# Veeryan/FDTD-solver-antennas

Measured on AMD Instinct MI355X. Metric: Mcells/s (Yee cells x steps / s), higher is better.
Workload: dtype f32; 1 GPU; NS: 300x300x60 2.45 GHz patch on FR-4 (fixed scene), CPML-10, 1 lumped port(s), NF2FF surfaces (record); cells=5400000, operator=classes, parallelism=single GPU, fields_finite=True

## Files before the change

### fdtd-solver-antennas_amd/_capi.py

```python
from __future__ import annotations

import ctypes as C
import os
from typing import Optional

import numpy as np

_HERE = os.path.dirname(os.path.abspath(__file__))
HIP_LIB_NAME = "libfdtd_hip.so"

ABI_SYMBOLS = [
    "fdtd_version", "fdtd_device_count", "fdtd_backend", "fdtd_create", "fdtd_destroy",
    "fdtd_last_error", "fdtd_set_operator_raw", "fdtd_set_operator_classes", "fdtd_build_operator",
    "fdtd_operator_form", "fdtd_get_operator", "fdtd_set_cpml",
    "fdtd_set_mur", "fdtd_set_signal", "fdtd_add_source", "fdtd_add_probe", "fdtd_get_probe",
    "fdtd_set_dft", "fdtd_add_dft_box", "fdtd_get_dft_box", "fdtd_set_recorder", "fdtd_rec_transform", "fdtd_run", "fdtd_run_profiled",
    "fdtd_get_step", "fdtd_energy", "fdtd_p2p_export", "fdtd_p2p_attach", "fdtd_p2p_selftest", "fdtd_p2p_detach", "fdtd_p2p_link_info", "fdtd_schedule_info", "fdtd_comm_unique_id", "fdtd_comm_init", "fdtd_comm_nranks", "fdtd_link", "fdtd_run_linked", "fdtd_half_step",
    "fdtd_halo_get", "fdtd_halo_put", "fdtd_get_field", "fdtd_set_field", "fdtd_farfield",
]

SHEET_SYMBOLS = ["fdtd_sheet_set", "fdtd_sheet_get"]
SHEET_MAX_K = 8
DEBYE_SYMBOLS = ["fdtd_debye_set", "fdtd_debye_get"]
DEBYE_MAX_K = 8
DEBYE_MAX_MEDIA = 8
LORENTZ_SYMBOLS = ["fdtd_lorentz_set", "fdtd_lorentz_get"]
LORENTZ_MAX_K = 4
LORENTZ_MAX_MEDIA = 8
LUMPED_SYMBOLS = ["fdtd_lumped_set", "fdtd_lumped_get"]
MAGNETIC_SYMBOLS = ["fdtd_magnetic_set", "fdtd_magnetic_get"]
MAGNETIC_MAX_CLASSES = 255
TRAFFIC_SYMBOLS = ["fdtd_traffic_info"]
VOXEL_SYMBOLS = ["fdtd_voxelize"]
CONFORMAL_SYMBOLS = ["fdtd_conformal_set", "fdtd_conformal_get", "fdtd_voxel_fractions"]
SAR_SYMBOLS = ["fdtd_sar_local", "fdtd_sar_average"]
PLANEWAVE_SYMBOLS = ["fdtd_planewave_set"]
MAX_BOXES = 64


class FdtdDesc(C.Structure):
    _fields_ = [("nx", C.c_int32), ("ny", C.c_int32), ("nz", C.c_int32),
                ("k0", C.c_int32), ("nk", C.c_int32),
                ("rank", C.c_int32), ("world", C.c_int32),
                ("device", C.c_int32), ("max_steps", C.c_int32),
                ("flags", C.c_uint32), ("dt", C.c_double)]


class FdtdProfile(C.Structure):
    _fields_ = [("ms_total", C.c_double), ("ms_update_e", C.c_double), ("ms_update_h", C.c_double),
                ("launches_e", C.c_int32), ("launches_h", C.c_int32),
                ("steps", C.c_int32), ("fused", C.c_int32), ("ms_event_overhead", C.c_double)]


FLAG_KERNEL_AUTO, FLAG_KERNEL_DIRECT, FLAG_KERNEL_WAVEFRONT, FLAG_KERNEL_RESIDENT, FLAG_KERNEL_MASK = 0, 1, 5, 6, 0xF
FLAG_OVERLAP_ON, FLAG_OVERLAP_OFF, FLAG_LOOPBACK = 0x20, 0x40, 0x80
KIND_V, KIND_I = 0, 1
PHASE_E, PHASE_H = 0, 1
HALO_H_UP, HALO_E_DOWN = 0, 1

_vp, _i, _i64p = C.c_void_p, C.c_int, C.POINTER(C.c_int64)


def bind(lib: C.CDLL) -> C.CDLL:
    p = C.c_void_p
    sig = {
        "fdtd_version": (C.c_int, []),
# ... 90 lines not shown
        "fdtd_magnetic_get": (C.c_int, [p, C.c_int, p, p]),
    }
    assert sorted(magnetic_sig) == sorted(MAGNETIC_SYMBOLS)
    for name, (res, args) in magnetic_sig.items():
        fn = getattr(lib, name, None)
        if fn is not None:
            fn.restype = res
            fn.argtypes = args
    traffic_sig = {"fdtd_traffic_info": (C.c_int, [p, p, C.POINTER(C.c_int32), C.POINTER(C.c_int64)])}
    assert sorted(traffic_sig) == sorted(TRAFFIC_SYMBOLS)
    for name, (res, args) in traffic_sig.items():
        fn = getattr(lib, name, None)
        if fn is not None:
            fn.restype = res
            fn.argtypes = args
    voxel_sig = {
        "fdtd_voxelize": (C.c_int, [C.c_int, C.c_int, C.c_int, C.c_int, p, C.c_int, p, C.c_int, p, C.c_double, p, p]),
    }
    assert sorted(voxel_sig) == sorted(VOXEL_SYMBOLS)
    for name, (res, args) in voxel_sig.items():
        fn = getattr(lib, name, None)
        if fn is not None:
            fn.restype = res
            fn.argtypes = args
    conformal_sig = {
        "fdtd_conformal_set": (C.c_int, [p, C.c_int, p, p, p]),
        "fdtd_conformal_get": (C.c_int, [p, p, p]),
        "fdtd_voxel_fractions": (C.c_int, [C.c_int, C.c_int, C.c_int, C.c_int, p, C.c_int, p, C.c_int, p, C.c_double, C.c_double,
                                           C.c_int, p, C.c_int64, p, p, p]),
    }
# ... 29 lines not shown

def has_planewave(lib: C.CDLL) -> bool:
    return all(hasattr(lib, n) for n in PLANEWAVE_SYMBOLS)


def has_conformal(lib: C.CDLL) -> bool:
    return all(hasattr(lib, n) for n in CONFORMAL_SYMBOLS)


def has_voxelize(lib: C.CDLL) -> bool:
    return all(hasattr(lib, n) for n in VOXEL_SYMBOLS)


def has_traffic_info(lib: C.CDLL) -> bool:
    return all(hasattr(lib, n) for n in TRAFFIC_SYMBOLS)


def has_magnetic(lib: C.CDLL) -> bool:
    return all(hasattr(lib, n) for n in MAGNETIC_SYMBOLS)


def has_lumped(lib: C.CDLL) -> bool:
    return all(hasattr(lib, n) for n in LUMPED_SYMBOLS)


def has_dispersion(lib: C.CDLL) -> bool:
    return all(hasattr(lib, n) for n in DEBYE_SYMBOLS)


def has_lorentz(lib: C.CDLL) -> bool:
# ... 23 lines not shown
    lib = bind(C.CDLL(path))
    if lib_dir is None:
        _hip_lib = lib
    return lib


def _ptr(a: Optional[np.ndarray]):
    return None if a is None else a.ctypes.data_as(C.c_void_p)


def _arr(a, dtype):
    return np.ascontiguousarray(a, dtype=dtype)


class FdtdError(RuntimeError):
    pass


class Engine:

    def __init__(self, lib: C.CDLL, nx: int, ny: int, nz: int, dt: float, *, k0: int = 0,
                 nk: Optional[int] = None, rank: int = 0, world: int = 1, device: int = 0,
                 max_steps: int = 0, flags: int = 0):
        self.lib = lib
        nk = nz - k0 if nk is None else nk
        self.desc = FdtdDesc(nx, ny, nz, k0, nk, rank, world, device, max_steps, flags, dt)
        self._ctx = C.c_void_p()
        rc = lib.fdtd_create(C.byref(self.desc), C.byref(self._ctx))
        if rc != 0:
            msg = lib.fdtd_last_error(None)
            raise FdtdError(f"fdtd_create failed ({rc}): {msg.decode() if msg else ''}")
        self.nx, self.ny, self.nz, self.k0, self.nk = nx, ny, nz, k0, nk
        self._keep = []

    def _ck(self, rc: int, what: str):
        if rc != 0:
            msg = self.lib.fdtd_last_error(self._ctx)
            raise FdtdError(f"{what} failed ({rc}): {msg.decode() if msg else ''}")

    def close(self):
        if self._ctx:
            self.lib.fdtd_destroy(self._ctx)
            self._ctx = C.c_void_p()

    def __del__(self):
        try:
            self.close()
        except Exception:
            pass

    @property
    def backend(self) -> str:
        return self.lib.fdtd_backend().decode()
# ... 140 lines not shown
        return bid.value

    def get_dft_box(self, bid: int):
        lo, hi = np.zeros(3, np.int32), np.zeros(3, np.int32)
        self._ck(self.lib.fdtd_get_dft_box(self._ctx, bid, None, _ptr(lo), _ptr(hi)), "get_dft_box")
        ext = hi - lo + 1
        if np.any(ext <= 0):
            return np.zeros((self.nfreq, 0, 0, 0), np.complex128), lo, hi
        out = np.zeros((self.nfreq, ext[2], ext[1], ext[0], 2), np.float64)
        self._ck(self.lib.fdtd_get_dft_box(self._ctx, bid, _ptr(out), _ptr(lo), _ptr(hi)), "get_dft_box")
        return out[..., 0] + 1j * out[..., 1], lo, hi

    def run(self, nsteps: int):
        self._ck(self.lib.fdtd_run(self._ctx, int(nsteps)), "run")

    def run_profiled(self, nsteps: int) -> FdtdProfile:
        prof = FdtdProfile()
        self._ck(self.lib.fdtd_run_profiled(self._ctx, int(nsteps), C.byref(prof)), "run_profiled")
        return prof

    @property
    def step(self) -> int:
        s = C.c_int64(0)
        self._ck(self.lib.fdtd_get_step(self._ctx, C.byref(s)), "get_step")
        return s.value

    def energy(self):
        s = np.zeros(2, np.float64)
        self._ck(self.lib.fdtd_energy(self._ctx, _ptr(s)), "energy")
        return float(s[0]), float(s[1])
# ... 391 lines not shown
```

### fdtd-solver-antennas_amd/csrc/api.hip

```cpp
#include <rccl/rccl.h>
#include <stdarg.h>
#include <stdio.h>
#include <stdlib.h>
#include <string.h>
#include <unistd.h>

#include <algorithm>
#include <mutex>
#include <chrono>
#include <unordered_map>
#include <vector>

#include "host_tables.hpp"
#include "../../include/fdtd_hip_traffic.h"
#include "kernel_common.hpp"

static thread_local std::string g_err;

int fdtd_fail(fdtd_ctx* c, int code, const char* fmt, ...) {
  char buf[768];
  va_list ap;
  va_start(ap, fmt);
  vsnprintf(buf, sizeof buf, fmt, ap);
  va_end(ap);
  if (c) c->err = buf; else g_err = buf;
  return code;
}

#define NCCLCK(c, expr)                                                                      \
// ... 207 lines not shown
  hipFree(c->cpcoef); hipFree(c->xc_tab); hipFree(c->pml_act);
  hipFree(c->xstamp);
  res_free(c);
  hipFree(c->wf_flags); hipFree(c->wf_err); hipFree(c->wf_flagsH); hipFree(c->wf_prb_sp); hipFree(c->wf_prb_blk); hipFree(c->wf_prb_rng);
  hipFree(c->wf_prbV_sp); hipFree(c->wf_prb_done);
  for (int n = 0; n < 12; ++n) hipFree(c->psi[n]);
  hipFree(c->d_mur);
  hipFree(c->rt_tw[0]); hipFree(c->rt_tw[1]); hipFree(c->rt_out);
  hipFree(c->sig); hipFree(c->src_off); hipFree(c->src_comp); hipFree(c->src_amp); hipFree(c->src_delay); hipFree(c->src_chain);
  for (int q = 0; q < c->nprobe; ++q) {
    hipFree((void*)c->probe[q].off); hipFree((void*)c->probe[q].comp); hipFree((void*)c->probe[q].w); hipFree(c->probe[q].series);
  }
  for (int b = 0; b < c->nbox; ++b) { hipFree(c->box[b].acc); hipFree(c->box[b].rec); }
  hipFree(c->d_probe); hipFree(c->d_box); hipFree(c->tw_v); hipFree(c->tw_i);
  hipFree(c->d_energy); hipFree(c->src_rng); hipFree(c->src_ids);
  sheet_free(c);
  lumped_free(c);
  planewave_free(c);
  media_free(&c->debye);
  media_free(&c->lorentz);
  magnetic_free(c);
  conformal_free(c);
  if (c->peer_lo && c->peer_lo_ipc) hipIpcCloseMemHandle(c->peer_lo);
  if (c->peer_hi && c->peer_hi_ipc) hipIpcCloseMemHandle(c->peer_hi);
  hipFree(c->mbox);
  if (c->ev_E) hipEventDestroy(c->ev_E);
  if (c->ev_H) hipEventDestroy(c->ev_H);
  if (c->ev_haloE) hipEventDestroy(c->ev_haloE);
  if (c->ev_haloH) hipEventDestroy(c->ev_haloH);
  if (!c->stream_shared) stream_give(c->d.device, c->stream);
// ... 1025 lines not shown
int fdtd_get_step(fdtd_ctx* c, int64_t* step) {
  if (!c || !step) return FDTD_E_ARG;
  *step = c->step;
  return FDTD_OK;
}

int fdtd_energy(fdtd_ctx* c, double sums[2]) {
  if (!c || !sums) return FDTD_E_ARG;
  HIPCK(c, hipSetDevice(c->d.device));
  launch_energy(c, c->stream);
  HIPCK(c, hipStreamSynchronize(c->stream));
  HIPCK(c, hipMemcpy(sums, c->d_energy, 2 * sizeof(double), hipMemcpyDeviceToHost));
  return FDTD_OK;
}

int fdtd_half_step(fdtd_ctx* c, int phase) {
  int r = check_ready(c);
  if (r) return r;
  if (c->p.p2p) return fdtd_fail(c, FDTD_E_STATE, "fdtd_half_step drives an external halo transport; detach the p2p transport first");
  HIPCK(c, hipSetDevice(c->d.device));
  hipStream_t s = c->stream;
  c->mur_pre_step = -1;
  if (phase == FDTD_PHASE_E) {
    launch_mur(c, 0, s);
    launch_update_E(c, 0, c->d.nk, c->step, false, false, s);
    launch_mur(c, 1, s);
    launch_mur(c, 2, s);
    launch_post(c, FDTD_KIND_V, c->step, true, s);
    launch_dft(c, FDTD_KIND_V, c->step, s);
    launch_debye(c, s);
// ... 520 lines not shown
```

### fdtd-solver-antennas_amd/csrc/fdtd_ctx.h

```cpp
#pragma once
#include <hip/hip_runtime.h>
#include <stdint.h>
#include <algorithm>
#include <map>
#include <string>
#include <utility>
#include <vector>

#include "../../include/fdtd_hip.h"

#define FDTD_MAX_PROBES 64
#define FDTD_MAX_BOXES 64
#define ENERGY_BLOCKS 1024
#ifndef FDTD_BLOCK
#define FDTD_BLOCK 256
#endif
#ifndef FDTD_E_MINBLOCKS
#define FDTD_E_MINBLOCKS 7
#endif
#ifndef FDTD_H_MINBLOCKS
#define FDTD_H_MINBLOCKS 7
#endif
#ifndef FDTD_WF_AUTO_MIB
#define FDTD_WF_AUTO_MIB 256
// ... 65 lines not shown
  unsigned wf_wait_bias;
  unsigned* wf_flagsH; const int* wf_prb_sp; const int* wf_prb_blk; const int2* wf_prb_rng;
  const int* wf_prbV_sp; unsigned* wf_prb_done;
  int nt;
  const int2* src_rng;
  const int* src_ids;
  int nsrc; const int* src_off; const int8_t* src_comp; const float* src_amp; const int* src_delay;
  int src_dense_ok;
  const unsigned* src_chain;
  const float* sig; int nsig;
  const struct DevProbe* probes; int nprobe; int max_steps;
  const MurDev* mur;
  int mur_nbx;
  int mur_nb;
  int mur_direct;
};

struct DevProbe { int kind, n; const int* off; const int8_t* comp; const float* w; double* series; };
struct DevBox   { int kind, comp; int lo[3]; int ni, nj, nkk; double* acc; long npts; float* rec;  };

struct MurFace { int on; float coeff; int n; };

struct ResHost {
  bool built = false;
  int nzt = 0, nstrips = 0, nblocks = 0;
  int* d_kt = nullptr; int* d_jt = nullptr;
  float* gx = nullptr; unsigned tag = 0;
  int2* d_src_rng = nullptr; int* d_src_ids = nullptr;
  int2* d_prb_rng = nullptr; int4* d_prb_cells = nullptr; int* d_slot0 = nullptr;
  float* stage = nullptr; int nslots = 1, chunk_cap = 0;
  int* err = nullptr;
// ... 85 lines not shown
  int nsrc = 0; int* src_off = nullptr; int8_t* src_comp = nullptr; float* src_amp = nullptr; int* src_delay = nullptr;
  unsigned* src_chain = nullptr;
  int src_max_per_strip_plane = 0;
  std::vector<int> h_src_off; std::vector<int8_t> h_src_comp; std::vector<float> h_src_amp; std::vector<int> h_src_delay;
  int nprobe = 0; DevProbe probe[FDTD_MAX_PROBES] = {}; DevProbe* d_probe = nullptr;
  bool iprb_pending = false;
  int nfreq = 0, every = 0, nsamples = 0; double *tw_v = nullptr, *tw_i = nullptr;
  bool recorder = false;
  int nbox = 0; DevBox box[FDTD_MAX_BOXES] = {}; DevBox* d_box = nullptr;
  int32_t box_lo[FDTD_MAX_BOXES][3] = {}, box_hi[FDTD_MAX_BOXES][3] = {};
  long box_maxpts[2] = {0, 0};
  double* rt_tw[2] = {nullptr, nullptr}; std::vector<double> rt_tw_host[2]; int rt_next = 0;
  double* rt_out = nullptr; size_t rt_out_bytes = 0;
  int64_t step = 0;
  double* d_energy = nullptr;
  hipStream_t stream = nullptr, comm_stream = nullptr;
  bool stream_shared = false;
  hipEvent_t ev_E = nullptr, ev_H = nullptr, ev_haloE = nullptr, ev_haloH = nullptr;
  bool haloE_pending = false, haloH_pending = false;
  void* comm = nullptr;
  int rccl_inline_mode = -1;
  fdtd_ctx* link_lo = nullptr;
  fdtd_ctx* link_hi = nullptr;
  bool haloE_issued = false, haloH_issued = false;
  bool tables_dirty = true;
  int launch_failed = 0;
  hipEvent_t kev0 = nullptr, kev1 = nullptr;
  EdgeList sheet;
  int sheet_K = 0, sheet_ncls = 0;
  float* sheet_ib = nullptr; float* sheet_alpha = nullptr; float* sheet_b = nullptr;
// ... 30 lines not shown
int upload_metric_tables(fdtd_ctx* c, const float* emet, const float* hmet);
void launch_update_E(fdtd_ctx* c, int k_begin, int k_end, long long step, bool fused, bool probe_block, hipStream_t s, bool mur_post = false);
void launch_update_H(fdtd_ctx* c, int k_begin, int k_end, long long step, bool probe_block, hipStream_t s, MurStep mur = MUR_NONE,
                     bool v_probes = true);
int launch_step_wf(fdtd_ctx* c, long long step, hipStream_t s, int nsteps, int lag);
int wf_multi_max(const fdtd_ctx* c);
int wf_lag_for(const fdtd_ctx* c);
void launch_p2p_prime(fdtd_ctx* c, hipStream_t s);
void launch_probes(fdtd_ctx* c, long long step, hipStream_t s);
int build_mur_table(fdtd_ctx* c);
void launch_mur(fdtd_ctx* c, int mode, hipStream_t s);
void launch_post(fdtd_ctx* c, int kind, long long step, bool sources, hipStream_t s);
void launch_dft(fdtd_ctx* c, int kind, long long step, hipStream_t s);
void launch_rec_dft(const float* rec, long npts, int ns, int nfreq, const double* d_tw, double* d_out, hipStream_t s);
void launch_energy(fdtd_ctx* c, hipStream_t s);
void choose_tiling(fdtd_ctx* c);
int chip_cus(int device);
bool res_possible(fdtd_ctx* c, const char** why);
int res_prepare(fdtd_ctx* c, int max_chunk);
int launch_resident(fdtd_ctx* c, long long step, int nsteps, hipStream_t s);
void res_free(fdtd_ctx* c);
enum Correction { CORR_SHEET, CORR_DEBYE, CORR_LORENTZ, CORR_LUMPED, CORR_MAGNETIC, CORR_CONFORMAL, CORR_PLANEWAVE, CORR_COUNT };
int correction_single_slab(fdtd_ctx* c, Correction which);
inline int fdtd_fail_hip(fdtd_ctx* c, const char* who, hipError_t e) {
  return fdtd_fail(c, e == hipErrorOutOfMemory ? FDTD_E_NOMEM : FDTD_E_DEVICE, "%s: %s", who, hipGetErrorString(e));
}
template <typename T>
inline hipError_t to_device(T** dst, const std::vector<T>& v) {
  hipFree(*dst); *dst = nullptr;
  hipError_t e = hipMalloc((void**)dst, std::max<size_t>(v.size(), 1) * sizeof(T));
// ... 38 lines not shown
```

### fdtd-solver-antennas_amd/csrc/kernel_common.hpp

```cpp
#pragma once
#include "fdtd_ctx.h"

namespace {

__device__ __forceinline__ float4 ld4(const float* p) { return *reinterpret_cast<const float4*>(p); }
__device__ __forceinline__ void st4(float* p, const float4& v) { *reinterpret_cast<float4*>(p) = v; }
__device__ __forceinline__ float4 ldo4(const float* base, const unsigned e) {
  return *reinterpret_cast<const float4*>(reinterpret_cast<const char*>(base) + (e << 2));
}
__device__ __forceinline__ float ldo1(const float* base, const unsigned e) {
  return *reinterpret_cast<const float*>(reinterpret_cast<const char*>(base) + (e << 2));
}
typedef float v4f_nt __attribute__((ext_vector_type(4)));
__device__ __forceinline__ void st4s(const int nt, float* p, const float4& v) {
  if (nt) {
    v4f_nt t = {v.x, v.y, v.z, v.w};
    __builtin_nontemporal_store(t, reinterpret_cast<v4f_nt*>(p));
  } else {
    *reinterpret_cast<float4*>(p) = v;
  }
}
__device__ __forceinline__ void sto4s(const int nt, float* base, const unsigned e, const float4& v) {
  st4s(nt, reinterpret_cast<float*>(reinterpret_cast<char*>(base) + (e << 2)), v);
}
// ... 106 lines not shown
}
__device__ __forceinline__ void sto1_dev(float* base, const unsigned e, const float v) {
  __builtin_amdgcn_raw_buffer_store_b32(__float_as_uint(v), dev_buf(base), (int)(e << 2), 0, 16);
}
__device__ __forceinline__ void wf_publish(const DevParams& p, unsigned* flags, const int k, const int strip, const int pb, const unsigned target) {
  asm volatile("s_waitcnt vmcnt(0)" ::: "memory");
  __syncthreads();
  if (threadIdx.x == 0)
    __hip_atomic_store(flags + ((size_t)k * p.nstrips + strip) * p.nbs + pb, target, __ATOMIC_RELAXED, __HIP_MEMORY_SCOPE_AGENT);
}
__device__ __forceinline__ int sload_int(const int* q) {
  int v;
  asm volatile("s_load_dword %0, %1, 0x0\n\ts_waitcnt lgkmcnt(0)" : "=s"(v) : "s"(q));
  return v;
}
__device__ __forceinline__ void wf_poll(const DevParams& p, const unsigned* f, const unsigned target) {
  const unsigned long long t0 = wall_clock64();
  unsigned seen;
  while ((seen = __hip_atomic_load(f, __ATOMIC_RELAXED, __HIP_MEMORY_SCOPE_AGENT)) < target) {
    __builtin_amdgcn_s_sleep(2);
    if (__hip_atomic_load(p.wf_err, __ATOMIC_RELAXED, __HIP_MEMORY_SCOPE_AGENT) != 0) break;
    if ((unsigned long long)wall_clock64() - t0 > p.wf_limit) {
      if (atomicCAS(p.wf_err, 0, 1) == 0) {
        const long de = f - p.wf_flags, dh = f - p.wf_flagsH;
        const bool is_e = de >= 0 && de < (long)p.nk * p.nstrips * p.nbs;
        p.wf_err[1] = (int)(is_e ? de : dh); p.wf_err[2] = (int)target; p.wf_err[3] = (int)seen; p.wf_err[4] = (int)blockIdx.x;
        p.wf_err[5] = is_e ? 0 : (dh >= 0 && dh < (long)p.nk * p.nstrips * p.nbs ? 1 : 2);
      }
      break;
    }
// ... 373 lines not shown
```

### fdtd-solver-antennas_amd/csrc/kernels.hip

```cpp
#include <hip/hip_ext.h>
#include <algorithm>
#include <cmath>
#include <map>
#include <mutex>
#include <vector>

#include "kernel_common.hpp"

namespace {

struct MurVals { float x0, x1; };
__device__ __forceinline__ float4 mur_post4(const float c, const float4& v, const float4& s) {
  return make_float4(__builtin_fmaf(c, v.x, s.x), __builtin_fmaf(c, v.y, s.y), __builtin_fmaf(c, v.z, s.z), __builtin_fmaf(c, v.w, s.w));
}
template <int PHASE, bool DEV = false>
__device__ __forceinline__ void mur_post_inline(const DevParams& p, const MurDev& m, const int k, const int j, const int i0, MurVals& mv,
                                                const float4& vx, const float4& vy, const float4& vz, const int par = 0) {
  auto ld = [](const float* q, const int o) { return DEV ? ldb4_dev(dev_buf(q), (unsigned)o << 2, 0u) : ld4(q + o); };
  auto st = [](float* q, const int o, const float4& v) { if (DEV) sto4_dev(q, (unsigned)o, v); else st4(q + o, v); };
#pragma unroll
  for (int fi = 0; fi < 6; ++fi) {
    const MurDevFace& f = m.f[fi];
    if (!f.on) continue;
    const int a = fi >> 1, pc = par * f.cdn;
// ... 549 lines not shown
}

#ifdef FDTD_XCD_TRACE
#define FDTD_XCD_TRACE_MAX 65536
__device__ unsigned long long g_xcd_trace[2 * FDTD_XCD_TRACE_MAX * 4];
#endif
template <int COEF, bool PML, bool P2P, bool MULTI = false, bool MUR = false>
__global__ __launch_bounds__(FDTD_BLOCK, (P2P || MUR) ? FDTD_WF_MINBLOCKS - 1 : FDTD_WF_MINBLOCKS) void k_step(const DevParams p, const long long step0, const int lag, const unsigned wf_target0,
                                                                        const unsigned nbp, const FastDiv fd_2m, const int down, const unsigned nmain,
                                                                        const FastDiv fd_per, const MurDev mur, const MurH mh) {
  static_assert(!(MUR && P2P), "Mur faces inside one launch: single slabs only");
  extern __shared__ float2 s_lut[];
  __shared__ float4 s_psi[(PML && FDTD_PSI_STAGE) ? FDTD_BLOCK * PSI_SLOTS : 3 * FDTD_BLOCK];
  __shared__ float s_xc[(PML && FDTD_PSI_STAGE) ? 3 * XC_MAX : 1];
  __shared__ SrcStage s_src;
  unsigned b = blockIdx.x;
  long long step = step0;
  unsigned wf_target = wf_target0, ts = 0u;
  if (MULTI) {
    ts = fd_div(b, fd_per);
    b -= ts * fd_per.d;
    step += ts;
    wf_target += ts;
  }
  const unsigned x = b & 7u, pos = b >> 3;
  if (b >= nmain) {
    if ((int)(b - nmain) < p.nprobe) wf_probe_tail<MULTI>(p, (int)(b - nmain), step, wf_target, reinterpret_cast<double*>(s_psi));
    return;
  }
  if (p.xstamp && b < 8u && threadIdx.x == 0) p.xstamp[p.xstamp_n + b] = wall_clock64();
// ... 27 lines not shown
#endif
  if (!is_h) body_E<COEF, PML, true, P2P, true, MUR, MULTI>(p, (int)strip, k, pb, step, s_lut, s_psi, s_xc, s_src, wf_target, MUR ? &mur : nullptr, ts ? wf_target - 1u : 0u);
  else body_H<COEF == 0, PML, P2P, true, MULTI, MUR>(p, (int)strip, k, pb, step, s_psi, s_xc, wf_target, ts ? wf_target - 1u : 0u, MUR ? &mh : nullptr);
  if (p.xstamp && threadIdx.x == 0) p.xstamp[b] = wall_clock64();
#ifdef FDTD_XCD_TRACE
  if (threadIdx.x == 0 && b < FDTD_XCD_TRACE_MAX) {
    unsigned xid;
    asm volatile("s_getreg_b32 %0, hwreg(HW_REG_XCC_ID)" : "=s"(xid));
    unsigned long long* const slot = g_xcd_trace + ((size_t)(step & 1) * FDTD_XCD_TRACE_MAX + b) * 4;
    slot[0] = t_begin; slot[1] = wall_clock64(); slot[2] = (xid & 7u) | (is_h ? 8u : 0u) | 16u; slot[3] = (unsigned long long)step;
  }
#endif
}

__global__ __launch_bounds__(FDTD_BLOCK) void k_mur(const DevParams p, const MurDev m, const int mode) {
  const int fi = blockIdx.y >> 1, t = blockIdx.y & 1;
  const MurDevFace& f = m.f[fi];
  if (!f.on) return;
  const int s = blockIdx.x * FDTD_BLOCK + threadIdx.x;
  if (s >= f.du * f.dv) return;
  const int iv = s / f.du, iu = s - iv * f.du;
  const int stride[3] = {1, p.P, p.plane};
  int pos[3];
  pos[f.a] = f.b; pos[f.ua] = iu; pos[f.va] = iv;
  const int comp = f.comp[t];
  float* V = p.V[comp];
  const int ob = pos[0] + pos[1] * p.P + pos[2] * p.plane;
  const int oi = ob + (f.in - f.b) * stride[f.a];
  const int ci = iv * f.cs + iu;
  if (mode == 0) {
// ... 54 lines not shown
    const float* F = (pr.kind == FDTD_KIND_V ? p.V[pr.comp[e]] : p.I[pr.comp[e]]);
    s = fma((double)pr.w[e], (double)F[pr.off[e]], s);
  }
  red[threadIdx.x] = s;
  __syncthreads();
  for (int w = FDTD_BLOCK / 2; w > 0; w >>= 1) {
    if ((int)threadIdx.x < w) red[threadIdx.x] += red[threadIdx.x + w];
    __syncthreads();
  }
  if (threadIdx.x == 0) pr.series[step] = red[0];
}

__global__ __launch_bounds__(FDTD_BLOCK) void k_dft(const DevParams p, const int kind, const DevBox* __restrict__ boxes,
                                                    const int nfreq, const int every, const int nsamples,
                                                    const double* __restrict__ tw_v, const double* __restrict__ tw_i, const long long step) {
  if (step % every != 0) return;
  const long long smp = step / every;
  if (smp >= nsamples) return;
  const DevBox bx = boxes[blockIdx.y];
  if ((kind >= 0 && bx.kind != kind) || bx.npts == 0) return;
  const float* F = (bx.kind == FDTD_KIND_V ? p.V[bx.comp] : p.I[bx.comp]);
  const double* w = (bx.kind == FDTD_KIND_V ? tw_v : tw_i) + smp * nfreq * 2;
  for (long pt = (long)blockIdx.x * FDTD_BLOCK + threadIdx.x; pt < bx.npts; pt += (long)gridDim.x * FDTD_BLOCK) {
    const int ii = (int)(pt % bx.ni);
    const long r = pt / bx.ni;
    const int jj = (int)(r % bx.nj), kk = (int)(r / bx.nj);
    const double v = (double)F[(bx.lo[2] + kk) * p.plane + (bx.lo[1] + jj) * p.P + bx.lo[0] + ii];
    for (int f = 0; f < nfreq; ++f) {
      double* a = bx.acc + ((long)f * bx.npts + pt) * 2;
      a[0] = fma(v, w[2 * f], a[0]);
      a[1] = fma(v, w[2 * f + 1], a[1]);
    }
  }
}

__global__ __launch_bounds__(FDTD_BLOCK) void k_rec(const DevParams p, const int kind, const DevBox* __restrict__ boxes,
                                                    const int every, const int nsamples, const long long step) {
  const long long smp = step / every;
  if (step % every != 0 || smp >= nsamples) return;
  const DevBox bx = boxes[blockIdx.y];
  if ((kind >= 0 && bx.kind != kind) || bx.npts == 0) return;
  const float* F = (bx.kind == FDTD_KIND_V ? p.V[bx.comp] : p.I[bx.comp]);
  float* dst = bx.rec + (size_t)smp * bx.npts;
  for (long pt = (long)blockIdx.x * FDTD_BLOCK + threadIdx.x; pt < bx.npts; pt += (long)gridDim.x * FDTD_BLOCK) {
    const int ii = (int)(pt % bx.ni);
    const long r = pt / bx.ni;
    const int jj = (int)(r % bx.nj), kk = (int)(r / bx.nj);
    dst[pt] = F[(bx.lo[2] + kk) * p.plane + (bx.lo[1] + jj) * p.P + bx.lo[0] + ii];
  }
}

template <int NF>
__global__ __launch_bounds__(FDTD_BLOCK) void k_rec_dft(const float* __restrict__ rec, const long npts, const int ns, const int nfreq,
                                                        const int f0, const double* __restrict__ tw, double* __restrict__ out) {
// ... 2 lines not shown
  double ar[NF], ai[NF];
#pragma unroll
  for (int q = 0; q < NF; ++q) ar[q] = ai[q] = 0.0;
  for (int s = 0; s < ns; ++s) {
    const double v = (double)rec[(size_t)s * npts + pt];
    const double* w = tw + ((size_t)s * nfreq + f0) * 2;
#pragma unroll
    for (int q = 0; q < NF; ++q)
      if (f0 + q < nfreq) { ar[q] = fma(v, w[2 * q], ar[q]); ai[q] = fma(v, w[2 * q + 1], ai[q]); }
  }
#pragma unroll
  for (int q = 0; q < NF; ++q)
    if (f0 + q < nfreq) { double* o = out + ((size_t)(f0 + q) * npts + pt) * 2; o[0] = ar[q]; o[1] = ai[q]; }
}

__global__ __launch_bounds__(FDTD_BLOCK) void k_energy(const DevParams p, double* out, double* part, unsigned* arrived) {
  __shared__ double rv[FDTD_BLOCK], ri[FDTD_BLOCK];
  double sv = 0.0, si = 0.0;
  const int n4 = p.nloc / 4;
  for (int t = blockIdx.x * FDTD_BLOCK + threadIdx.x; t < n4; t += gridDim.x * FDTD_BLOCK) {
#pragma unroll
    for (int c = 0; c < 3; ++c) {
      const float4 v = ld4(p.V[c] + 4 * t), i = ld4(p.I[c] + 4 * t);
      sv += (double)v.x * v.x + (double)v.y * v.y + (double)v.z * v.z + (double)v.w * v.w;
      si += (double)i.x * i.x + (double)i.y * i.y + (double)i.z * i.z + (double)i.w * i.w;
    }
  }
  rv[threadIdx.x] = sv; ri[threadIdx.x] = si;
  __syncthreads();
  for (int w = FDTD_BLOCK / 2; w > 0; w >>= 1) {
    if ((int)threadIdx.x < w) { rv[threadIdx.x] += rv[threadIdx.x + w]; ri[threadIdx.x] += ri[threadIdx.x + w]; }
    __syncthreads();
  }
  __shared__ unsigned last;
  if (threadIdx.x == 0) {
    part[2 * blockIdx.x] = rv[0]; part[2 * blockIdx.x + 1] = ri[0];
    __threadfence();
    last = atomicAdd(arrived, 1u) == gridDim.x - 1u ? 1u : 0u;
  }
  __syncthreads();
  if (!last) return;
  __threadfence();
  double sv2 = 0.0, si2 = 0.0;
  for (unsigned b = threadIdx.x; b < gridDim.x; b += FDTD_BLOCK) {
    sv2 += __hip_atomic_load(part + 2 * b, __ATOMIC_RELAXED, __HIP_MEMORY_SCOPE_AGENT);
    si2 += __hip_atomic_load(part + 2 * b + 1, __ATOMIC_RELAXED, __HIP_MEMORY_SCOPE_AGENT);
  }
  rv[threadIdx.x] = sv2; ri[threadIdx.x] = si2;
  __syncthreads();
  for (int w = FDTD_BLOCK / 2; w > 0; w >>= 1) {
    if ((int)threadIdx.x < w) { rv[threadIdx.x] += rv[threadIdx.x + w]; ri[threadIdx.x] += ri[threadIdx.x + w]; }
    __syncthreads();
  }
  if (threadIdx.x == 0) { out[0] = rv[0]; out[1] = ri[0]; *arrived = 0u; }
}

}

void choose_tiling(fdtd_ctx* c) {
  const int P4 = c->p.P4, ny = c->p.ny;
  const unsigned sel = c->d.flags & FDTD_FLAG_KERNEL_MASK;
  const bool wf_big = (size_t)(c->d.nk + 2) * c->plane * 6 * sizeof(float) > ((size_t)FDTD_WF_AUTO_MIB << 20);
  const bool wf_like = wf_big && sel != FDTD_FLAG_KERNEL_DIRECT;
  int best = 1; double best_cost = 1e30;
  for (int tys = 4; tys <= 40; ++tys) {
    const int rows = tys < ny ? tys : ny;
    const int t = rows * P4;
    const int nbs = (t + FDTD_BLOCK - 1) / FDTD_BLOCK;
    const double halo = 1.0 / tys * 0.15;
// ... 526 lines not shown
  const dim3 grid((unsigned)((npts + FDTD_BLOCK - 1) / FDTD_BLOCK)), block(FDTD_BLOCK);
  for (int f0 = 0; f0 < nfreq; f0 += 8)
    hipLaunchKernelGGL((k_rec_dft<8>), grid, block, 0, s, rec, npts, ns, nfreq, f0, d_tw, d_out);
}

void launch_post(fdtd_ctx* c, int kind, long long step, bool sources, hipStream_t s) {
  hipLaunchKernelGGL(k_post, dim3(1), dim3(FDTD_BLOCK), 0, s, c->p, kind, sources ? 1 : 0, step);
}

void launch_energy(fdtd_ctx* c, hipStream_t s) {
  const unsigned nblk = (unsigned)std::max<size_t>(1, std::min<size_t>(ENERGY_BLOCKS, (c->nloc / 4 + FDTD_BLOCK - 1) / FDTD_BLOCK));
  hipLaunchKernelGGL(k_energy, dim3(nblk), dim3(FDTD_BLOCK), 0, s, c->p, c->d_energy, c->d_energy + 2,
                     reinterpret_cast<unsigned*>(c->d_energy + 2 + 2 * ENERGY_BLOCKS));
}

#ifdef FDTD_XCD_TRACE
extern "C" int fdtd_debug_xcd_trace(long long step, unsigned long long* out) {
  if (step < 0) {
    void* q = nullptr;
    if (hipGetSymbolAddress(&q, HIP_SYMBOL(g_xcd_trace)) != hipSuccess) return -3;
    return hipMemset(q, 0, sizeof(unsigned long long) * 2 * FDTD_XCD_TRACE_MAX * 4) == hipSuccess ? 0 : -3;
  }
  return hipMemcpyFromSymbol(out, HIP_SYMBOL(g_xcd_trace), (size_t)FDTD_XCD_TRACE_MAX * 4 * sizeof(unsigned long long),
                             (size_t)(step & 1) * FDTD_XCD_TRACE_MAX * 4 * sizeof(unsigned long long)) == hipSuccess ? 0 : -3;
}
#endif
```

### fdtd-solver-antennas_amd/csrc/resident.hip

```cpp
#include <hip/hip_ext.h>
#include <algorithm>
#include <vector>

#include "kernel_common.hpp"

namespace {

constexpr int RES_MAX_SRC = 128;
constexpr int RES_MAX_PRB = 256;
#ifndef RES_POLL_SLEEP
#define RES_POLL_SLEEP 0
#endif

struct ResDev {
  int nzt, nstrips;
  const int* kt;
  const int* jt;
  float* gx;
  int* err; unsigned long long limit;
  const int2* src_rng; const int* src_ids;
  const int2* prb_rng; const int4* prb_cells;
  float* stage; int nslots;
  const DevBox* boxes; int nbox, every, nsamples;
  int mur_on[6]; float mur_c[6];
// ... 117 lines not shown
    if (!in) { if (!store) ps[q] = make_float4(0.f, 0.f, 0.f, 0.f); continue; }
    if (store) st4(arr[q] + o, ps[q]); else ps[q] = ld4(arr[q] + o);
  }
}

template <int COEF, bool MUR, bool PML>
__global__ __launch_bounds__(FDTD_BLOCK, 2) void k_resident(const DevParams p, const ResDev r) {
  __shared__ float4 sV[3][FDTD_BLOCK], sI[3][FDTD_BLOCK];
  __shared__ float4 sO[MUR ? 3 : 1][MUR ? FDTD_BLOCK : 1];
  __shared__ int s_sthr[RES_MAX_SRC], s_sdel[RES_MAX_SRC];
  __shared__ float s_samp[RES_MAX_SRC], s_sval[RES_MAX_SRC];
  __shared__ signed char s_ssel[RES_MAX_SRC];
  __shared__ int s_pthr[RES_MAX_PRB], s_pslot[RES_MAX_PRB];
  __shared__ signed char s_psel[RES_MAX_PRB];

  const unsigned b = blockIdx.x, nblocks = gridDim.x;
#ifdef FDTD_RES_TRACE
  const unsigned long long tr_begin = wall_clock64();
  unsigned long long tr_ew = 0, tr_ec = 0, tr_hw = 0, tr_hc = 0, tr_setup = 0;
#endif
  const int zt = (int)(b / (unsigned)r.nstrips), strip = (int)(b - (unsigned)zt * (unsigned)r.nstrips);
  const int k0 = r.kt[zt], ZT = r.kt[zt + 1] - k0, j0 = r.jt[strip], R = r.jt[strip + 1] - j0;
  const int P4 = p.P4, RP = R * P4, nth = ZT * RP;
  const int t = (int)threadIdx.x;
  const bool valid = t < nth;
  const int tt = valid ? t : 0;
  const int kk = tt / RP, rem = tt - kk * RP, rr = rem / P4, g = rem - rr * P4;
  const int k = k0 + kk, j = j0 + rr, i0 = 4 * g;
  const int off = k * p.plane + j * p.P + i0;
  const DevRsrc rs = dev_buf(r.gx);
// ... 232 lines not shown
    unsigned long long* q = g_res_trace + 8 * b;
    q[0] = tr_ew; q[1] = tr_ec; q[2] = tr_hw; q[3] = tr_hc; q[4] = wall_clock64() - tr_begin; q[5] = tr_setup; q[6] = (unsigned long long)r.nsteps;
  }
#endif
  if constexpr (PML) { res_psi_io(pm, p.psiE, psE, true); res_psi_io(pm, p.psiH, psH, true); }
  if (valid) {
    st4(p.V[0] + off, vx); st4(p.V[1] + off, vy); st4(p.V[2] + off, vz);
    st4(p.I[0] + off, ix); st4(p.I[1] + off, iy); st4(p.I[2] + off, iz);
  }
}

__global__ __launch_bounds__(FDTD_BLOCK) void k_res_probes(const DevParams p, const float* __restrict__ stage, const int nslots,
                                                           const int* __restrict__ slot0, const long long step0) {
  __shared__ double red[FDTD_BLOCK];
  const long long step = step0 + blockIdx.y;
  if (step < 0 || step >= p.max_steps) return;
  const DevProbe pr = p.probes[blockIdx.x];
  const float* cells = stage + (size_t)blockIdx.y * nslots + slot0[blockIdx.x];
  double s = 0.0;
  for (int e = threadIdx.x; e < pr.n; e += FDTD_BLOCK) s = fma((double)pr.w[e], (double)cells[e], s);
  red[threadIdx.x] = s;
  __syncthreads();
  for (int w = FDTD_BLOCK / 2; w > 0; w >>= 1) {
    if ((int)threadIdx.x < w) red[threadIdx.x] += red[threadIdx.x + w];
    __syncthreads();
  }
  if (threadIdx.x == 0) pr.series[step] = red[0];
}

template <int COEF, bool MUR, bool PML>
const void* res_kernel() { return reinterpret_cast<const void*>(&k_resident<COEF, MUR, PML>); }
// ... 186 lines not shown
```

### fdtd-solver-antennas_amd/simulation.py

```python
from __future__ import annotations

import os
from dataclasses import dataclass, field
from typing import List, Optional, Sequence
import numpy as np

from .constants import C0, EPS0, MU0, ETA0
from .grid import RectGrid
from .scene import VoxelScene
from .ecoperator import build_operator, ECOperator, metric_lists, pack_metric_tables, lumped_overrides, LumpedEdge
from . import sheet as _sheet
from . import lumped as _lumped
from . import dispersion as _disp
from . import lorentz as _lorentz
from . import magnetic as _magnetic
from . import conformal as _conformal
from . import sar as _sar
from . import planewave as _planewave
from .cpml import CPMLSpec, build_cpml
from .excitation import gauss_pulse, dft_twiddles
from .nf2ff import NF2FFBox, calc_nf2ff
from . import _capi
from ._capi import Engine, KIND_V, KIND_I

# ... 611 lines not shown
                "K": d.K, "poles": int(sum(m.K for m in d.media)), "edges": len(d),
                "fit_errors": {"tan_delta": max([m.fit_info["tan_delta_error"] for m in d.media if m.fit_info] or [None], key=lambda v: v or 0),
                               "eps": max([m.fit_info["eps_error"] for m in d.media if m.fit_info] or [None], key=lambda v: v or 0)},
                "box_edges": [int(np.prod(w.shape)) for w in d.w]}

    def run(self, *, max_steps: Optional[int] = None, check_every: int = 200, verbose: int = 0,
            allreduce=None, log=print) -> RunStats:
        import time
        e = self.engine
        total = self.nr_ts if max_steps is None else min(max_steps, self.nr_ts)
        emax, stats = 0.0, RunStats()
        t0 = time.perf_counter()
        done = e.step
        fresh = done == 0
        comm = getattr(self, "comm", None)
        while done < total:
            n = min(check_every, total - done)
            if self.external_transport is not None:
                self.external_transport.run_steps(e, n)
            elif self.world > 1 and fresh and done == 0 and comm is not None and comm.transport == "auto":
                code, why = 0, ""
                try:
                    e.run(n)
                except _capi.FdtdError as exc:
                    why = str(exc)
                    low = why.lower()
                    code = 1 if "wavefront schedule" in low else 2 if ("p2p" in low or "nccl" in low or "rccl" in low) else 3
                worst = int(round(float(np.max(comm.allreduce_max(np.array([float(code)]))))))
                if worst == 3:
                    raise _capi.FdtdError(why or f"rank {self.rank}: another rank's engine failed in the first timesteps of the decomposed run")
                if worst:
# ... 87 lines not shown
```

Baseline: 81900 Mcells/s.

## Run to the energy criterion on-device with an asynchronous check window

Adds fdtd_run_until, which enqueues up to four step chunks ahead, each followed by a fused energy-plus-stop kernel that writes a device stop flag. Every kernel checks that flag and exits early, so the host no longer blocks on an energy readback after each check interval. This removes the per-chunk host round trip and keeps the GPU fed. In exchange it adds a load of the stop flag at the start of every kernel launch and more complex rollback bookkeeping for steps enqueued past the stopping chunk.

```diff
diff --git a/fdtd-solver-antennas_amd/_capi.py b/fdtd-solver-antennas_amd/_capi.py
--- a/fdtd-solver-antennas_amd/_capi.py
+++ b/fdtd-solver-antennas_amd/_capi.py
@@ -31,6 +31,8 @@
 MAGNETIC_SYMBOLS = ["fdtd_magnetic_set", "fdtd_magnetic_get"]
 MAGNETIC_MAX_CLASSES = 255
 TRAFFIC_SYMBOLS = ["fdtd_traffic_info"]
+UNTIL_SYMBOLS = ["fdtd_run_until"]
+E_UNSUPPORTED = -5
 VOXEL_SYMBOLS = ["fdtd_voxelize"]
 CONFORMAL_SYMBOLS = ["fdtd_conformal_set", "fdtd_conformal_get", "fdtd_voxel_fractions"]
 SAR_SYMBOLS = ["fdtd_sar_local", "fdtd_sar_average"]
@@ -50,6 +52,17 @@
     _fields_ = [("ms_total", C.c_double), ("ms_update_e", C.c_double), ("ms_update_h", C.c_double),
                 ("launches_e", C.c_int32), ("launches_h", C.c_int32),
                 ("steps", C.c_int32), ("fused", C.c_int32), ("ms_event_overhead", C.c_double)]
+
+
+class FdtdUntil(C.Structure):
+    _fields_ = [("max_steps", C.c_int32), ("check_every", C.c_int32), ("min_steps", C.c_int32), ("reserved", C.c_int32),
+                ("end_criteria", C.c_double), ("w_v", C.c_double), ("w_i", C.c_double)]
+
+
+class FdtdUntilResult(C.Structure):
+    _fields_ = [("steps", C.c_int32), ("stopped", C.c_int32), ("checks", C.c_int32), ("reserved", C.c_int32),
+                ("sum_v", C.c_double), ("sum_i", C.c_double),
+                ("energy", C.c_double), ("energy_max", C.c_double), ("ratio", C.c_double)]
 
 
 FLAG_KERNEL_AUTO, FLAG_KERNEL_DIRECT, FLAG_KERNEL_WAVEFRONT, FLAG_KERNEL_RESIDENT, FLAG_KERNEL_MASK = 0, 1, 5, 6, 0xF
@@ -170,6 +183,13 @@
         if fn is not None:
             fn.restype = res
             fn.argtypes = args
+    until_sig = {"fdtd_run_until": (C.c_int, [p, C.POINTER(FdtdUntil), C.POINTER(FdtdUntilResult)])}
+    assert sorted(until_sig) == sorted(UNTIL_SYMBOLS)
+    for name, (res, args) in until_sig.items():
+        fn = getattr(lib, name, None)
+        if fn is not None:
+            fn.restype = res
+            fn.argtypes = args
     voxel_sig = {
         "fdtd_voxelize": (C.c_int, [C.c_int, C.c_int, C.c_int, C.c_int, p, C.c_int, p, C.c_int, p, C.c_double, p, p]),
     }
@@ -229,6 +249,10 @@
 
 def has_traffic_info(lib: C.CDLL) -> bool:
     return all(hasattr(lib, n) for n in TRAFFIC_SYMBOLS)
+
+
+def has_run_until(lib: C.CDLL) -> bool:
+    return all(hasattr(lib, n) for n in UNTIL_SYMBOLS)
 
 
 def has_magnetic(lib: C.CDLL) -> bool:
@@ -282,7 +306,11 @@
 
 
 class FdtdError(RuntimeError):
-    pass
+    code = None
+
+
+class FdtdUnsupported(FdtdError):
+    """FDTD_E_UNSUPPORTED: the call was refused with the context untouched."""
 
 
 class Engine:
@@ -304,7 +332,9 @@
     def _ck(self, rc: int, what: str):
         if rc != 0:
             msg = self.lib.fdtd_last_error(self._ctx)
-            raise FdtdError(f"{what} failed ({rc}): {msg.decode() if msg else ''}")
+            exc = (FdtdUnsupported if rc == E_UNSUPPORTED else FdtdError)(f"{what} failed ({rc}): {msg.decode() if msg else ''}")
+            exc.code = rc
+            raise exc
 
     def close(self):
         if self._ctx:
@@ -475,6 +505,14 @@
     def run(self, nsteps: int):
         self._ck(self.lib.fdtd_run(self._ctx, int(nsteps)), "run")
 
+    def run_until(self, max_steps: int, check_every: int, min_steps: int, end_criteria: float, w_v: float, w_i: float) -> FdtdUntilResult:
+        if not has_run_until(self.lib):
+            raise FdtdError(f"this library ({self.backend}) has no fdtd_run_until")
+        arg = FdtdUntil(int(max_steps), int(check_every), int(min_steps), 0, float(end_criteria), float(w_v), float(w_i))
+        res = FdtdUntilResult()
+        self._ck(self.lib.fdtd_run_until(self._ctx, C.byref(arg), C.byref(res)), "run_until")
+        return res
+
     def run_profiled(self, nsteps: int) -> FdtdProfile:
         prof = FdtdProfile()
         self._ck(self.lib.fdtd_run_profiled(self._ctx, int(nsteps), C.byref(prof)), "run_profiled")
diff --git a/fdtd-solver-antennas_amd/csrc/api.hip b/fdtd-solver-antennas_amd/csrc/api.hip
--- a/fdtd-solver-antennas_amd/csrc/api.hip
+++ b/fdtd-solver-antennas_amd/csrc/api.hip
@@ -13,6 +13,7 @@
 
 #include "host_tables.hpp"
 #include "../../include/fdtd_hip_traffic.h"
+#include "../../include/fdtd_hip_until.h"
 #include "kernel_common.hpp"
 
 static thread_local std::string g_err;
@@ -250,6 +251,9 @@
   for (int b = 0; b < c->nbox; ++b) { hipFree(c->box[b].acc); hipFree(c->box[b].rec); }
   hipFree(c->d_probe); hipFree(c->d_box); hipFree(c->tw_v); hipFree(c->tw_i);
   hipFree(c->d_energy); hipFree(c->src_rng); hipFree(c->src_ids);
+  hipFree(c->until_dev);
+  if (c->until_host) hipHostFree(c->until_host);
+  for (hipEvent_t e : c->until_ev) if (e) hipEventDestroy(e);
   sheet_free(c);
   lumped_free(c);
   planewave_free(c);
@@ -1305,6 +1309,98 @@
   return FDTD_OK;
 }
 
+namespace {
+constexpr int UNTIL_WINDOW = 4, UNTIL_RING = 8;
+static_assert(UNTIL_WINDOW + 2 <= UNTIL_RING, "the slots in flight and the stopping chunk's snapshot fit the ring");
+struct UntilDev { int stop, pad; double emax; UntilRecord rec; };
+struct UntilSlot { UntilRecord rec; int wf_err[8]; int res_err, pad; };
+struct UntilSnap { int64_t step, mur_pre_step; unsigned wf_epoch, res_tag; bool iprb_pending; int xcd_adapt_calls; };
+struct StopGuard { fdtd_ctx* c; ~StopGuard() { c->p.stop = nullptr; } };
+}
+
+int fdtd_run_until(fdtd_ctx* c, const fdtd_until* in, fdtd_until_result* out) {
+  int r = check_ready(c);
+  if (r) return r;
+  if (!in || !out || in->max_steps < 0 || in->check_every < 1) return fdtd_fail(c, FDTD_E_ARG, "run_until: max_steps >= 0, check_every >= 1");
+  memset(out, 0, sizeof *out);
+  out->ratio = 1.0;
+  if (c->d.world != 1 || c->p.p2p || c->comm || c->link_lo || c->link_hi)
+    return fdtd_fail(c, FDTD_E_UNSUPPORTED, "run_until: single slab only (world = 1, no p2p transport, communicator or linked contexts)");
+  HIPCK(c, hipSetDevice(c->d.device));
+  StepPlan pl;
+  if ((r = plan_schedule(c, false, &pl))) return r;
+  if (pl.kind != StepPlan::RESIDENT && pl.kind != StepPlan::ONE_LAUNCH)
+    return fdtd_fail(c, FDTD_E_UNSUPPORTED, "run_until: the resident schedule or one launch per timestep only (this context takes two launches per timestep: step it with fdtd_run and fdtd_energy)");
+  if (in->max_steps == 0) return FDTD_OK;
+  hipStream_t s = c->stream;
+  if (!c->until_dev) HIPCK(c, hipMalloc(&c->until_dev, sizeof(UntilDev)));
+  if (!c->until_host) HIPCK(c, hipHostMalloc(&c->until_host, UNTIL_RING * sizeof(UntilSlot), hipHostMallocDefault));
+  for (int q = 0; q < UNTIL_RING; ++q)
+    if (!c->until_ev[q]) HIPCK(c, hipEventCreateWithFlags(&c->until_ev[q], hipEventDisableTiming));
+  UntilDev* const dev = static_cast<UntilDev*>(c->until_dev);
+  UntilSlot* const host = static_cast<UntilSlot*>(c->until_host);
+  HIPCK(c, hipMemsetAsync(dev, 0, sizeof(UntilDev), s));
+  c->p.stop = &dev->stop;
+  StopGuard guard{c};
+
+  const int64_t step0 = c->step;
+  UntilSnap snap[UNTIL_RING];
+  int64_t done_at[UNTIL_RING];
+  UntilRecord last{};
+  int enq = 0, seen = 0, stop_chunk = -1, checks = 0;
+  bool dev_err = false;
+  auto consume = [&](int k) -> int {
+    HIPCK(c, hipEventSynchronize(c->until_ev[k % UNTIL_RING]));
+    const UntilSlot& sl = host[k % UNTIL_RING];
+    if (stop_chunk < 0 && sl.rec.done == done_at[k % UNTIL_RING] && sl.rec.live) {
+      last = sl.rec;
+      ++checks;
+      if (sl.rec.stop) stop_chunk = k;
+    }
+    if (sl.wf_err[0] || sl.res_err) dev_err = true;
+    return FDTD_OK;
+  };
+  int remaining = in->max_steps;
+  while (remaining > 0 && stop_chunk < 0 && !dev_err) {
+    while (seen < enq - UNTIL_WINDOW && stop_chunk < 0 && !dev_err) { if ((r = consume(seen))) return r; ++seen; }
+    if (stop_chunk >= 0 || dev_err) break;
+    const int n = std::min(in->check_every, remaining), q = enq % UNTIL_RING;
+    r = pl.kind == StepPlan::RESIDENT ? step_loop_res(c, pl, n, nullptr) : step_loop_wf(c, pl, n, nullptr);
+    if (r) { hipStreamSynchronize(s); return r; }
+    remaining -= n;
+    const UntilArgs a{(long long)c->step, (long long)in->min_steps, in->end_criteria, in->w_v, in->w_i};
+    launch_energy_until(c, a, &dev->emax, &dev->rec, &dev->stop, s);
+    memset(&host[q], 0, sizeof(UntilSlot));
+    HIPCK(c, hipMemcpyAsync(&host[q].rec, &dev->rec, sizeof(UntilRecord), hipMemcpyDeviceToHost, s));
+    if (c->wf_err) HIPCK(c, hipMemcpyAsync(host[q].wf_err, c->wf_err, sizeof host[q].wf_err, hipMemcpyDeviceToHost, s));
+    if (c->res.err) HIPCK(c, hipMemcpyAsync(&host[q].res_err, c->res.err, sizeof(int), hipMemcpyDeviceToHost, s));
+    HIPCK(c, hipEventRecord(c->until_ev[q], s));
+    snap[q] = UntilSnap{c->step, c->mur_pre_step, c->wf_epoch, c->res.tag, c->iprb_pending, c->xcd_adapt_calls};
+    done_at[q] = c->step;
+    ++enq;
+    if (c->xstamp_grid && c->xstamp_mode) {
+      while (seen < enq) { if ((r = consume(seen))) return r; ++seen; }
+      if ((stop_chunk < 0 || stop_chunk == enq - 1) && !dev_err) { if ((r = xcd_adapt(c))) return r; }
+      else { c->xstamp_grid = 0; c->xstamp_mode = 0; }
+    }
+  }
+  while (seen < enq) { if ((r = consume(seen))) return r; ++seen; }
+  HIPCK(c, hipStreamSynchronize(s));
+  if (stop_chunk >= 0 && stop_chunk < enq - 1) {
+    const UntilSnap& sn = snap[stop_chunk % UNTIL_RING];
+    c->step = sn.step; c->mur_pre_step = sn.mur_pre_step; c->wf_epoch = sn.wf_epoch; c->res.tag = sn.res_tag;
+    c->iprb_pending = sn.iprb_pending; c->xcd_adapt_calls = sn.xcd_adapt_calls;
+    c->xstamp_grid = 0; c->xstamp_mode = 0;
+  }
+  out->steps = (int32_t)(c->step - step0);
+  out->stopped = stop_chunk >= 0 ? 1 : 0;
+  out->checks = checks;
+  if (checks) { out->sum_v = last.sv; out->sum_i = last.si; out->energy = last.en; out->energy_max = last.emax; out->ratio = last.ratio; }
+  if ((r = launch_status(c))) return r;
+  if ((r = wf_check(c))) return r;
+  return res_check(c);
+}
+
 int fdtd_half_step(fdtd_ctx* c, int phase) {
   int r = check_ready(c);
   if (r) return r;
diff --git a/fdtd-solver-antennas_amd/csrc/fdtd_ctx.h b/fdtd-solver-antennas_amd/csrc/fdtd_ctx.h
--- a/fdtd-solver-antennas_amd/csrc/fdtd_ctx.h
+++ b/fdtd-solver-antennas_amd/csrc/fdtd_ctx.h
@@ -103,7 +103,11 @@
   int mur_nbx;
   int mur_nb;
   int mur_direct;
-};
+  const int* stop;
+};
+
+struct UntilRecord { long long done; double sv, si, en, emax, ratio; int stop, live; };
+struct UntilArgs { long long done, min_steps; double end_criteria, w_v, w_i; };
 
 struct DevProbe { int kind, n; const int* off; const int8_t* comp; const float* w; double* series; };
 struct DevBox   { int kind, comp; int lo[3]; int ni, nj, nkk; double* acc; long npts; float* rec;  };
@@ -219,6 +223,7 @@
   double* rt_out = nullptr; size_t rt_out_bytes = 0;
   int64_t step = 0;
   double* d_energy = nullptr;
+  void* until_dev = nullptr; void* until_host = nullptr; hipEvent_t until_ev[8] = {};
   hipStream_t stream = nullptr, comm_stream = nullptr;
   bool stream_shared = false;
   hipEvent_t ev_E = nullptr, ev_H = nullptr, ev_haloE = nullptr, ev_haloH = nullptr;
@@ -279,6 +284,7 @@
 void launch_dft(fdtd_ctx* c, int kind, long long step, hipStream_t s);
 void launch_rec_dft(const float* rec, long npts, int ns, int nfreq, const double* d_tw, double* d_out, hipStream_t s);
 void launch_energy(fdtd_ctx* c, hipStream_t s);
+void launch_energy_until(fdtd_ctx* c, const UntilArgs& a, double* emax, UntilRecord* rec, int* stop, hipStream_t s);
 void choose_tiling(fdtd_ctx* c);
 int chip_cus(int device);
 bool res_possible(fdtd_ctx* c, const char** why);
diff --git a/fdtd-solver-antennas_amd/csrc/kernel_common.hpp b/fdtd-solver-antennas_amd/csrc/kernel_common.hpp
--- a/fdtd-solver-antennas_amd/csrc/kernel_common.hpp
+++ b/fdtd-solver-antennas_amd/csrc/kernel_common.hpp
@@ -144,6 +144,7 @@
   asm volatile("s_load_dword %0, %1, 0x0\n\ts_waitcnt lgkmcnt(0)" : "=s"(v) : "s"(q));
   return v;
 }
+__device__ __forceinline__ bool stop_set(const DevParams& p) { return p.stop != nullptr && sload_int(p.stop) != 0; }
 __device__ __forceinline__ void wf_poll(const DevParams& p, const unsigned* f, const unsigned target) {
   const unsigned long long t0 = wall_clock64();
   unsigned seen;
diff --git a/fdtd-solver-antennas_amd/csrc/kernels.hip b/fdtd-solver-antennas_amd/csrc/kernels.hip
--- a/fdtd-solver-antennas_amd/csrc/kernels.hip
+++ b/fdtd-solver-antennas_amd/csrc/kernels.hip
@@ -587,6 +587,7 @@
   __shared__ float4 s_psi[(PML && FDTD_PSI_STAGE) ? FDTD_BLOCK * PSI_SLOTS : 3 * FDTD_BLOCK];
   __shared__ float s_xc[(PML && FDTD_PSI_STAGE) ? 3 * XC_MAX : 1];
   __shared__ SrcStage s_src;
+  if (stop_set(p)) return;
   unsigned b = blockIdx.x;
   long long step = step0;
   unsigned wf_target = wf_target0, ts = 0u;
@@ -644,6 +645,7 @@
 }
 
 __global__ __launch_bounds__(FDTD_BLOCK) void k_mur(const DevParams p, const MurDev m, const int mode) {
+  if (stop_set(p)) return;
   const int fi = blockIdx.y >> 1, t = blockIdx.y & 1;
   const MurDevFace& f = m.f[fi];
   if (!f.on) return;
@@ -728,7 +730,7 @@
 __global__ __launch_bounds__(FDTD_BLOCK) void k_dft(const DevParams p, const int kind, const DevBox* __restrict__ boxes,
                                                     const int nfreq, const int every, const int nsamples,
                                                     const double* __restrict__ tw_v, const double* __restrict__ tw_i, const long long step) {
-  if (step % every != 0) return;
+  if (step % every != 0 || stop_set(p)) return;
   const long long smp = step / every;
   if (smp >= nsamples) return;
   const DevBox bx = boxes[blockIdx.y];
@@ -751,7 +753,7 @@
 __global__ __launch_bounds__(FDTD_BLOCK) void k_rec(const DevParams p, const int kind, const DevBox* __restrict__ boxes,
                                                     const int every, const int nsamples, const long long step) {
   const long long smp = step / every;
-  if (step % every != 0 || smp >= nsamples) return;
+  if (step % every != 0 || smp >= nsamples || stop_set(p)) return;
   const DevBox bx = boxes[blockIdx.y];
   if ((kind >= 0 && bx.kind != kind) || bx.npts == 0) return;
   const float* F = (bx.kind == FDTD_KIND_V ? p.V[bx.comp] : p.I[bx.comp]);
@@ -784,7 +786,7 @@
     if (f0 + q < nfreq) { double* o = out + ((size_t)(f0 + q) * npts + pt) * 2; o[0] = ar[q]; o[1] = ai[q]; }
 }
 
-__global__ __launch_bounds__(FDTD_BLOCK) void k_energy(const DevParams p, double* out, double* part, unsigned* arrived) {
+__device__ __forceinline__ bool energy_sums(const DevParams& p, double* out, double* part, unsigned* arrived) {
   __shared__ double rv[FDTD_BLOCK], ri[FDTD_BLOCK];
   double sv = 0.0, si = 0.0;
   const int n4 = p.nloc / 4;
@@ -809,7 +811,7 @@
     last = atomicAdd(arrived, 1u) == gridDim.x - 1u ? 1u : 0u;
   }
   __syncthreads();
-  if (!last) return;
+  if (!last) return false;
   __threadfence();
   double sv2 = 0.0, si2 = 0.0;
   for (unsigned b = threadIdx.x; b < gridDim.x; b += FDTD_BLOCK) {
@@ -823,6 +825,23 @@
     __syncthreads();
   }
   if (threadIdx.x == 0) { out[0] = rv[0]; out[1] = ri[0]; *arrived = 0u; }
+  return threadIdx.x == 0;
+}
+__global__ __launch_bounds__(FDTD_BLOCK) void k_energy(const DevParams p, double* out, double* part, unsigned* arrived) {
+  energy_sums(p, out, part, arrived);
+}
+__global__ __launch_bounds__(FDTD_BLOCK) void k_energy_until(const DevParams p, double* out, double* part, unsigned* arrived, const UntilArgs a,
+                                                             double* emax_io, UntilRecord* rec, int* stop) {
+  if (stop_set(p)) return;
+  if (!energy_sums(p, out, part, arrived)) return;
+  const double sv = out[0], si = out[1];
+  const double en = a.w_v * sv + a.w_i * si;
+  const double emax = fmax(*emax_io, en);
+  const double ratio = emax > 0.0 ? en / emax : 1.0;
+  const int st = (a.end_criteria > 0.0 && a.done >= a.min_steps && ratio < a.end_criteria) ? 1 : 0;
+  *emax_io = emax;
+  rec->done = a.done; rec->sv = sv; rec->si = si; rec->en = en; rec->emax = emax; rec->ratio = ratio; rec->stop = st; rec->live = 1;
+  if (st) *stop = 1;
 }
 
 }
@@ -1379,6 +1398,12 @@
                      reinterpret_cast<unsigned*>(c->d_energy + 2 + 2 * ENERGY_BLOCKS));
 }
 
+void launch_energy_until(fdtd_ctx* c, const UntilArgs& a, double* emax, UntilRecord* rec, int* stop, hipStream_t s) {
+  const unsigned nblk = (unsigned)std::max<size_t>(1, std::min<size_t>(ENERGY_BLOCKS, (c->nloc / 4 + FDTD_BLOCK - 1) / FDTD_BLOCK));
+  hipLaunchKernelGGL(k_energy_until, dim3(nblk), dim3(FDTD_BLOCK), 0, s, c->p, c->d_energy, c->d_energy + 2,
+                     reinterpret_cast<unsigned*>(c->d_energy + 2 + 2 * ENERGY_BLOCKS), a, emax, rec, stop);
+}
+
 #ifdef FDTD_XCD_TRACE
 extern "C" int fdtd_debug_xcd_trace(long long step, unsigned long long* out) {
   if (step < 0) {
diff --git a/fdtd-solver-antennas_amd/csrc/resident.hip b/fdtd-solver-antennas_amd/csrc/resident.hip
--- a/fdtd-solver-antennas_amd/csrc/resident.hip
+++ b/fdtd-solver-antennas_amd/csrc/resident.hip
@@ -155,6 +155,7 @@
   __shared__ int s_pthr[RES_MAX_PRB], s_pslot[RES_MAX_PRB];
   __shared__ signed char s_psel[RES_MAX_PRB];
 
+  if (stop_set(p)) return;
   const unsigned b = blockIdx.x, nblocks = gridDim.x;
 #ifdef FDTD_RES_TRACE
   const unsigned long long tr_begin = wall_clock64();
@@ -417,7 +418,7 @@
                                                            const int* __restrict__ slot0, const long long step0) {
   __shared__ double red[FDTD_BLOCK];
   const long long step = step0 + blockIdx.y;
-  if (step < 0 || step >= p.max_steps) return;
+  if (step < 0 || step >= p.max_steps || stop_set(p)) return;
   const DevProbe pr = p.probes[blockIdx.x];
   const float* cells = stage + (size_t)blockIdx.y * nslots + slot0[blockIdx.x];
   double s = 0.0;
diff --git a/fdtd-solver-antennas_amd/simulation.py b/fdtd-solver-antennas_amd/simulation.py
--- a/fdtd-solver-antennas_amd/simulation.py
+++ b/fdtd-solver-antennas_amd/simulation.py
@@ -649,7 +649,32 @@
         done = e.step
         fresh = done == 0
         comm = getattr(self, "comm", None)
+        until = (_capi.has_run_until(self.lib) and self.world == 1 and self.external_transport is None and allreduce is None
+                 and not verbose and os.environ.get("FDTD_RUN_UNTIL", "") != "0")
         while done < total:
+            if until:
+                until = False
+                try:
+                    res = e.run_until(total - done, check_every, len(self.signal), self.end_criteria, EPS0, MU0)
+                except _capi.FdtdUnsupported:
+                    res = None
+                except _capi.FdtdError as exc:
+                    if not (fresh and ("wavefront schedule" in str(exc) or "resident schedule" in str(exc)) and stats.schedule_fallback is None):
+                        raise
+                    log(f"[fdtd-hip] {exc} — repeating the run under the two-launch schedule")
+                    e.close()
+                    e = self.build(self.lib, rank=self.rank, world=self.world, device=self.device, partition=self.partition,
+                                   flags=(self._build_flags & ~_capi.FLAG_KERNEL_MASK) | _capi.FLAG_KERNEL_DIRECT)
+                    stats.schedule_fallback = str(exc)
+                    done, emax = 0, 0.0
+                    continue
+                if res is not None:
+                    done += res.steps
+                    if res.checks:
+                        stats.energy_db = 10.0 * np.log10(max(res.ratio, 1e-300))
+                    stats.stopped_by_energy = bool(res.stopped)
+                    break
+                continue
             n = min(check_every, total - done)
             if self.external_transport is not None:
                 self.external_transport.run_steps(e, n)
diff --git a/include/fdtd_hip_until.h b/include/fdtd_hip_until.h
--- /dev/null
+++ b/include/fdtd_hip_until.h
@@ -0,0 +1,34 @@
+#ifndef FDTD_HIP_UNTIL_H
+#define FDTD_HIP_UNTIL_H
+
+#include <stdint.h>
+#include "fdtd_hip.h"
+
+#ifdef __cplusplus
+extern "C" {
+#endif
+
+typedef struct fdtd_until {
+  int32_t max_steps;
+  int32_t check_every;
+  int32_t min_steps;
+  int32_t reserved;
+  double end_criteria;
+  double w_v, w_i;
+} fdtd_until;
+
+typedef struct fdtd_until_result {
+  int32_t steps;
+  int32_t stopped;
+  int32_t checks;
+  int32_t reserved;
+  double sum_v, sum_i;
+  double energy, energy_max, ratio;
+} fdtd_until_result;
+
+int fdtd_run_until(fdtd_ctx* ctx, const fdtd_until* in, fdtd_until_result* out);
+
+#ifdef __cplusplus
+}
+#endif
+#endif
```

After: 81930 Mcells/s, median of 4. No clear change (+0.0%).
